# adamnelsonarcher/BB-OCR

Measured on AMD Instinct MI355X. Metric: book-page images/sec end-to-end (detect+recognize) @1280x960, higher is better.
Workload: dtype fp16

## Files before the change

bb-ocr_amd/csrc/conv_mfma.hip:

```cpp
#include "common.h"
#include "kernels.h"
#include <type_traits>
#include <utility>

__device__ __forceinline__ void lds_dma16(const void* gptr, const void* lds) {
    const unsigned la = (unsigned)(size_t)(const __attribute__((address_space(3))) void*)lds;
    asm volatile("s_mov_b32 m0, %1\n\ts_nop 0\n\tglobal_load_lds_dwordx4 %0, off" ::"v"(gptr), "s"(la) : "memory");
}

template <int EL, int MF, bool ADDUP = false>
__device__ __forceinline__ void conv_epilogue(const ConvArgs& a, f32x4 (&acc)[MF][4], int n, int nt, int oy0, int ox0, int wm, int wn, int fpr,
                                              int lane, int BN, int sub = 1, int sph = 0, int spw = 0) {
    const int g = lane >> 4, pl = lane & 15;
    const int cout0 = nt * BN + wn * 64 + g * 8;
    if (a.tail) {
        const float* tw = a.tail;
        const typename El<EL>::v8 w1f = *(const typename El<EL>::v8*)(a.tail_frag + lane * 8);
        float cb[8], b1r[4], w2a[4], w2b[4];
#pragma unroll
        for (int i = 0; i < 8; ++i) cb[i] = a.bias[(g & 1) * 8 + i];
#pragma unroll
        for (int r = 0; r < 4; ++r) { b1r[r] = tw[4 * g + r]; w2a[r] = tw[16 + 4 * g + r]; w2b[r] = tw[32 + 4 * g + r]; }
        const float b20 = tw[48], b21 = tw[49];
#pragma unroll
// ... 221 lines not shown
                            *(u32x4*)(op) = lo;
                            if (run1) *(u32x4*)(op + 32) = hi;
                        }
                    };
                    if (a.split_off) {
                        float mh[16], ml[16];
                        split_hi_lo(m, mh, ml);
                        store_pooled(mh, 0);
                        store_pooled(ml, a.split_off);
                    } else {
                        store_pooled(m, 0);
                    }
                } else {
                    store_frag(a.pool_out, prow, a.pool_cs, xb, POW, py < POH, m, false);
                }
            }
        }
    };
    if (fpr == 1) pooled(std::integral_constant<int, 1>{});
    else if (fpr == 2) pooled(std::integral_constant<int, 2>{});
    else pooled(std::integral_constant<int, 4>{});
}

template <int EL, int MF>
__device__ __forceinline__ void conv_epilogue_pool2x2_lean(const ConvArgs& a, f32x4 (&acc)[MF][4], int n, int oy0, int ox0, int wm, int lane,
                                                           int cout_base = 0) {
    static_assert(MF % 2 == 0, "fragment f and f + 1 are the two rows of a pooling window");
    const int g = lane >> 4, pl = lane & 15, odd = pl & 1;
    const int cout0 = cout_base + g * 8;
    const float sc = a.acc_scale;
    const float floor_v = (a.relu_out || a.pool_relu) ? 0.f : -__builtin_inff();
    float bsel[8];
#pragma unroll
    for (int q = 0; q < 2; ++q) {
        const f32x4 b4 = *(const f32x4*)(a.bias + cout0 + odd * 32 + q * 4);
        bsel[q * 4 + 0] = b4[0]; bsel[q * 4 + 1] = b4[1]; bsel[q * 4 + 2] = b4[2]; bsel[q * 4 + 3] = b4[3];
    }
    const int POH = a.OH >> 1, POW = a.OW >> 1;
    const int px = (ox0 + pl) >> 1;
#pragma unroll
    for (int f = 0; f < MF; f += 2) {
        const int py = (oy0 + wm * MF + f) >> 1;
        float o[8];
#pragma unroll
        for (int i = 0; i < 8; ++i) {
            const int i1 = 8 + i;
            float q0 = fmaxf(acc[f][i >> 2][i & 3], acc[f + 1][i >> 2][i & 3]);
            float q1 = fmaxf(acc[f][i1 >> 2][i1 & 3], acc[f + 1][i1 >> 2][i1 & 3]);
            q0 = fmaxf(q0, __int_as_float(__builtin_amdgcn_update_dpp(0, __float_as_int(q0), 0xB1 , 0xF, 0xF, true)));
            q1 = fmaxf(q1, __int_as_float(__builtin_amdgcn_update_dpp(0, __float_as_int(q1), 0xB1, 0xF, 0xF, true)));
            o[i] = fmaxf(fmaf(odd ? q1 : q0, sc, bsel[i]), floor_v);
        }
        const u32x4 pk = {El<EL>::pack2(o[0], o[1]), El<EL>::pack2(o[2], o[3]), El<EL>::pack2(o[4], o[5]), El<EL>::pack2(o[6], o[7])};
        uint16_t* op = (uint16_t*)a.pool_out + ((size_t)(n * POH + py) * POW + px) * a.pool_cs + cout0 + odd * 32;
        if (py < POH && px < POW) *(u32x4*)op = pk;
    }
}

template <int EL, int MF>
__device__ __forceinline__ void conv_epilogue_plain_lean(const ConvArgs& a, f32x4 (&acc)[MF][4], int n, int nt, int oy0, int ox0, int wm, int wn,
                                                         int fpr, int lane, int BN) {
    typedef short s16x2_t __attribute__((ext_vector_type(2)));
    const int g = lane >> 4, pl = lane & 15;
    const int cout0 = nt * BN + wn * 64 + g * 8;
    float bs[16];
#pragma unroll
    for (int h = 0; h < 2; ++h)
#pragma unroll
        for (int q = 0; q < 2; ++q) {
            const f32x4 b4 = *(const f32x4*)(a.bias + cout0 + h * 32 + q * 4);
            bs[h * 8 + q * 4 + 0] = b4[0]; bs[h * 8 + q * 4 + 1] = b4[1]; bs[h * 8 + q * 4 + 2] = b4[2]; bs[h * 8 + q * 4 + 3] = b4[3];
        }
    const bool relu = a.relu_out != 0;
    const bool inside = oy0 + a.TH <= a.OH && ox0 + a.TW <= a.OW;
    const s16x2_t z2 = {0, 0};
    const size_t lane_off = (size_t)(pl & 7) * a.out_cs + cout0 + (pl >> 3) * 32;
#pragma unroll
    for (int f = 0; f < MF; ++f) {
        const int F = wm * MF + f;
// ... 239 lines not shown
                typename El<EL>::v8 bq[MF];
#pragma unroll
                for (int f = 0; f < MF; ++f) bq[f] = *(const typename El<EL>::v8*)(pb + frag_off[f]);
#pragma unroll
                for (int f = 0; f < MF; ++f) {
#pragma unroll
                    for (int j = 0; j < 4; ++j) acc[f][j] = El<EL>::mfma(af[j], bq[f], acc[f][j]);
                }
                __builtin_amdgcn_sched_group_barrier(0x100, 4 + MF, 0);
                __builtin_amdgcn_sched_group_barrier(0x008, 4 * MF, 0);
                if (more) {
                    if (a.ntaps >= 3) stage_patch_store(c + 1, tap);
                    else if (tap == a.ntaps - 1) store_part(c + 1, P0{});
                }
                __syncthreads();
                if (++kx == a.KW) { kx = 0; ++ky; }
            }
        }
    }

    conv_epilogue<EL, MF>(a, acc, n, nt, oy0, ox0, wm, wn, fpr, lane, BN);
}

template <int EL, int WM, int WN, int MF, int NPB, int RING, int NPS = NPB * 64, bool FUSE1 = false, int NF = 4, int EPI = 0, int KS = 3>
__global__ void __launch_bounds__(WM * WN * 64, 2) conv3x3_dma_kernel(const ConvArgs a) {
    constexpr int NTAP = KS * KS, PAD = KS == 3 ? 1 : 0;
    static_assert((KS == 3 || KS == 2) && (KS == 3 || (!FUSE1 && EPI == 0)), "kernel size");
    constexpr int NW = WM * WN, NT = NW * 64, BN = WN * 64;
    static_assert(NW == 4, "one wave per 8-channel group of the patch");
    constexpr int WBUF = BN * 64, WPIECES = WBUF / 16, WPT = WPIECES / NT;
    static_assert(WPIECES % NT == 0 && (RING == 3 || RING == 4), "uniform DMA issue");
    constexpr int NP = NPS, PSLOTS = NTAP + 1 - RING;
    constexpr int PPER = (NPB + PSLOTS - 1) / PSLOTS;
    static_assert(NPS <= NPB * 64 && NPS > (NPB - 1) * 64 && NPS % 4 == 0, "patch size");
    static_assert(PSLOTS >= 1 && PPER * PSLOTS >= NPB, "patch does not fit the DMA schedule");
    extern __shared__ __attribute__((aligned(16))) unsigned char smem[];
    unsigned char* const wbuf = smem;
    unsigned char* const pbuf = smem + RING * WBUF;
    constexpr int patch_bytes = NP * 64;

    const int tid = threadIdx.x;
    const int lane = tid & 63;
    const int wave = __builtin_amdgcn_readfirstlane(tid >> 6);
    const int wm = wave / WN, wn = wave % WN;
    const int sub = a.sub;
    const int nk = a.nchunks * NTAP;
    const int fpr = FUSE1 ? 1 : a.TW >> 4;
    const int PW = FUSE1 ? 18 : a.PW;

    const int tile = xcd_remap(blockIdx.x, gridDim.x);
    struct Geo {
        int n, nt, oy0, ox0, sph, spw;
        const unsigned char* wsrc;
    };
    auto geom = [&](int id, Geo& g) {
        g.nt = id % a.ntiles_n;
        id /= a.ntiles_n;
        const int tx = id % a.tiles_x;
        id /= a.tiles_x;
        const int ty = id % a.tiles_y;
        int n = id / a.tiles_y;
        g.sph = 0; g.spw = 0;
        g.n = n;
        g.oy0 = ty * a.TH; g.ox0 = tx * a.TW;
        g.wsrc = (const unsigned char*)a.wpk + (size_t)g.nt * nk * WBUF;
    };
    int spix[NPB];
    const int pw_magic = (65536 + a.PW - 1) / a.PW;
    const int stack_magic = ((1 << 20) + a.stack) / (a.stack + 1);
    auto geom_pix = [&](const Geo& g) {
        const int iy0 = g.oy0 - PAD, ix0 = g.ox0 - PAD;
#pragma unroll
        for (int pb = 0; pb < NPB; ++pb) {
            const int pix = pb * 64 + lane;
            const int py = (pix * pw_magic) >> 16, px = pix - py * a.PW;
            int ly = iy0 + py;
            const int lx = ix0 + px;
            int sph = 0, spw = 0;
            bool rowok = ly >= 0;
            if (sub > 1) {
                const int vy = ly < 0 ? 0 : ly;
                const int q = (vy * stack_magic) >> 20;
                ly = vy - q * (a.stack + 1);
                sph = q / sub;
                spw = q - sph * sub;
                rowok = rowok && ly < a.stack && q < sub * sub;
            }
            const int iy = ly * sub + sph, ix = lx * sub + spw;
            spix[pb] = (py < a.PH && rowok && iy < a.H && lx >= 0 && ix < a.W) ? (g.n * a.H + iy) * a.W + ix : -1;
        }
    };
    Geo cur;
    geom(tile, cur);
    if constexpr (!FUSE1) geom_pix(cur);

    auto issue_p = [&](int sp, int chunk, int par, auto pb_c) {
        constexpr int pb = decltype(pb_c)::value;
        const int c = chunk * 32;
        const bool s0 = c < a.C0;
        const uint16_t* src = s0 ? a.in0 : a.in1;
        const int cs = s0 ? a.in0_cs : a.in1_cs;
        const int cb = (s0 ? c : c - a.C0) + wave * 8;
        const uint16_t* gp = sp >= 0 ? src + (size_t)sp * cs + cb : (const uint16_t*)a.zero;
        if ((pb + 1) * 64 <= NPS || pb * 64 + lane < NPS)
            lds_dma16(gp, pbuf + par * patch_bytes + (wave * NP + pb * 64) * 16);
    };
    auto issue_w = [&](const unsigned char* slice, int slot) {
#pragma unroll
        for (int p0 = 0; p0 < WPIECES; p0 += NT) lds_dma16(slice + (size_t)(p0 + tid) * 16, wbuf + slot * WBUF + (p0 + wave * 64) * 16);
    };
    int frag_off[MF];
#pragma unroll
    for (int f = 0; f < MF; ++f) {
        const int F = wm * MF + f;
        const int fr = F / fpr, fc = F - fr * fpr;
        frag_off[f] = (fr * PW + fc * 16) * 16;
    }
    const int lane_patch_off = ((lane >> 4) * NP + (lane & 15)) * 16;
    const int lane_w_off = wn * 4 * 1024 + lane * 16;

    struct Sched {
        static constexpr int pcnt(int tap) {
            if (FUSE1 || tap >= PSLOTS) return 0;
            const int base = NPB / PSLOTS, extra = NPB % PSLOTS;
            return base + (tap < extra ? 1 : 0);
        }
        static constexpr int pfirst(int tap) { int s = 0; for (int t = 0; t < tap; ++t) s += pcnt(t); return s; }
        static constexpr int wcnt(bool more, int tap) { return (more || tap < NTAP - (RING - 1)) ? WPT : 0; }
        static constexpr int younger(bool more, int tap) {
            int nv = wcnt(more, tap) + (more ? pcnt(tap) : 0);
            for (int back = 1; back <= RING - 2; ++back) {
                const int t = tap - back;
                const bool m = t >= 0 ? more : true;
                const int tt = t >= 0 ? t : t + NTAP;
                const int pc = m ? pcnt(tt) : 0;
                nv += (back == RING - 2) ? pc : (wcnt(m, tt) + pc);
            }
            return nv;
        }
    };
    static_assert(FUSE1 || Sched::pfirst(NTAP) == NPB, "patch DMA schedule must cover the patch");

#pragma unroll
    for (int i = 0; i < RING - 1; ++i)
        if (i < nk) issue_w(cur.wsrc + (size_t)i * WBUF, i);
    if constexpr (!FUSE1) {
        [&]<int... PB>(std::integer_sequence<int, PB...>) { (issue_p(spix[PB], 0, 0, std::integral_constant<int, PB>{}), ...); }(std::make_integer_sequence<int, NPB>{});
    } else {
        static_assert(!FUSE1 || (RING == 3 && BN == 64 && NPS == 324), "fused conv1_1 producer: 16x16 tiles, 3-deep ring of 4 KB slices");
        u32x2* const rgbp = (u32x2*)(wbuf + 2 * WBUF);
        const uint8_t* rgb = (const uint8_t*)a.in0;
        const float m0 = 0.485f * 255.0f, m1 = 0.456f * 255.0f, m2 = 0.406f * 255.0f;
        const float s0 = 0.229f * 255.0f, s1 = 0.224f * 255.0f, s2 = 0.225f * 255.0f;
        static_assert(NT == 256, "two patch pixels per thread");
        int pq[2];
        bool on_canvas[2];
        unsigned int cr[2], cg[2], cb[2];
#pragma unroll
        for (int it = 0; it < 2; ++it) {
            const int p = tid + it * NT;
            const int py = p / 20, px = p - py * 20;
            const int iy = cur.oy0 - 2 + py, ix = cur.ox0 - 2 + px;
            pq[it] = p;
            on_canvas[it] = p < 400 && iy >= 0 && iy < a.H && ix >= 0 && ix < a.W;
            const bool on_page = on_canvas[it] && iy < a.rgb_H && ix < a.rgb_W;
            const uint8_t* q = rgb + (on_page ? ((size_t)(cur.n * a.rgb_H + iy) * a.rgb_W + ix) * 3 : (size_t)cur.n * a.rgb_H * a.rgb_W * 3);
            cr[it] = q[0]; cg[it] = q[1]; cb[it] = q[2];
            if (!on_page) { cr[it] = 0u; cg[it] = 0u; cb[it] = 0u; }
        }
        typename El<EL>::v8 w1[4];
#pragma unroll
        for (int j = 0; j < 4; ++j) w1[j] = *(const typename El<EL>::v8*)(a.c11_w + ((size_t)j * 64 + lane) * 8);
        const int g = lane >> 4, pl = lane & 15;
        f32x4 b1[4];
#pragma unroll
        for (int h = 0; h < 2; ++h)
#pragma unroll
            for (int q4 = 0; q4 < 2; ++q4) b1[h * 2 + q4] = *(const f32x4*)(a.c11_b + h * 32 + g * 8 + q4 * 4);
        __builtin_amdgcn_sched_barrier(0);
#pragma unroll
        for (int it = 0; it < 2; ++it) {
            if (pq[it] < 400) {
                u32x2 v = {0u, 0u};
                if (on_canvas[it]) {
                    v[0] = El<EL>::pack2(((float)cr[it] - m0) / s0, ((float)cg[it] - m1) / s1);
                    v[1] = El<EL>::pack2(((float)cb[it] - m2) / s2, 0.f);
                }
                rgbp[pq[it]] = v;
            }
        }
        __syncthreads();
        auto frag_geo = [&](int fi, int& pp, int& py, int& px) {
            pp = fi * 16 + pl;
            py = pp / 18;
            px = pp - py * 18;
        };
#pragma unroll
        for (int b3 = 0; b3 < 2; ++b3) {
            typename El<EL>::v8 bfr[3];
            int pps[3], pys[3], pxs[3];
#pragma unroll
            for (int q = 0; q < 3; ++q) {
                const int fi = wave + (b3 * 3 + q) * NW;
                frag_geo(fi < 21 ? fi : 20, pps[q], pys[q], pxs[q]);
                const int pc = pps[q] < 324 ? pys[q] * 20 + pxs[q] : 0;
                const int t0 = 2 * g, t1 = t0 + 1;
                const u32x2 a0 = rgbp[pc + (t0 / 3) * 20 + (t0 % 3)];
                const u32x2 a1 = rgbp[pc + (t1 / 3) * 20 + (t1 % 3)];
                const u32x2 t8 = rgbp[pc + 2 * 20 + 2];
                const unsigned int x = g == 0 ? (t8[0] << 16) : (g == 1 ? (t8[1] << 16) : 0u);
                const unsigned int y = g == 0 ? (t8[0] & 0xffff0000u) : 0u;
                bfr[q] = __builtin_bit_cast(typename El<EL>::v8, (u32x4){a0[0], a0[1] | x, a1[0], a1[1] | y});
            }
            f32x4 d[3][4];
#pragma unroll
            for (int q = 0; q < 3; ++q)
#pragma unroll
                for (int j = 0; j < 4; ++j) d[q][j] = El<EL>::mfma(w1[j], bfr[q], b1[j]);
#pragma unroll
            for (int q = 0; q < 3; ++q) {
                const int fi = wave + (b3 * 3 + q) * NW;
                const int pp = pps[q];
                const int iy = cur.oy0 - 1 + pys[q], ix = cur.ox0 - 1 + pxs[q];
                const bool inside = iy >= 0 && iy < a.H && ix >= 0 && ix < a.W;
                const float cap = inside ? __builtin_inff() : 0.f;
                if (fi < 21 && pp < 324) {
#pragma unroll
                    for (int h = 0; h < 2; ++h) {
                        u32x4 o;
#pragma unroll
                        for (int i = 0; i < 4; ++i) {
                            const int k = h * 8 + i * 2;
                            const float x0 = __builtin_amdgcn_fmed3f(d[q][k >> 2][k & 3], 0.f, cap), x1 = __builtin_amdgcn_fmed3f(d[q][(k + 1) >> 2][(k + 1) & 3], 0.f, cap);
                            o[i] = El<EL>::pack2(x0, x1);
                        }
                        *(u32x4*)(pbuf + h * patch_bytes + (g * NP + pp) * 16) = o;
                    }
                }
            }
        }
    }
    asm volatile("s_waitcnt vmcnt(0) lgkmcnt(0)\n\ts_barrier" ::: "memory");

    int wslot = 0, par = 0;
    const unsigned char* wp = cur.wsrc + (size_t)(RING - 1) * WBUF;
    f32x4 acc[MF][4];
#pragma unroll
    for (int f = 0; f < MF; ++f)
#pragma unroll
        for (int j = 0; j < 4; ++j) acc[f][j] = (f32x4){0.f, 0.f, 0.f, 0.f};
    static_assert(MF % 2 == 0 && MF >= 4, "B fragments are scheduled in pairs, four ahead");
    typename El<EL>::v8 pre[4];
    auto step = [&](auto tap_c, auto more_c, int c) {
        constexpr int tap = decltype(tap_c)::value;
        constexpr bool MORE = decltype(more_c)::value;
        constexpr int ky = tap / KS, kx = tap % KS;
        const unsigned char* wb = wbuf + wslot * WBUF + lane_w_off;
        const unsigned char* pb = pbuf + par * patch_bytes + lane_patch_off + (ky * PW + kx) * 16;
        typename El<EL>::v8 af[NF], bq[MF];
#pragma unroll
        for (int j = 0; j < NF; ++j) af[j] = *(const typename El<EL>::v8*)(wb + j * 1024);
        if constexpr (tap == 0) {
#pragma unroll
            for (int f = 0; f < 4; ++f) bq[f] = *(const typename El<EL>::v8*)(pb + frag_off[f]);
// ... 31 lines not shown
            __builtin_amdgcn_sched_barrier(0);
        }
        asm volatile("s_waitcnt vmcnt(%0)\n\ts_barrier" ::"n"(Sched::younger(MORE, tap)) : "memory");
        wslot = wslot + 1 == RING ? 0 : wslot + 1;
    };
    auto relu_patch = [&](int c) {
        if (!((c * 32 < a.C0) ? a.relu_in0 : a.relu_in1)) return;
        const s16x8 z = {0, 0, 0, 0, 0, 0, 0, 0};
        s16x8* pp = (s16x8*)(pbuf + par * patch_bytes);
#pragma unroll
        for (int i = 0; i < (NP * 4 + NT - 1) / NT; ++i) {
            const int k = tid + i * NT;
            if ((i + 1) * NT <= NP * 4 || k < NP * 4) pp[k] = __builtin_elementwise_max(pp[k], z);
        }
        asm volatile("s_waitcnt lgkmcnt(0)\n\ts_barrier" ::: "memory");
    };
    auto chunk = [&](auto more_c, int c) {
        relu_patch(c);
        [&]<int... T>(std::integer_sequence<int, T...>) { (step(std::integral_constant<int, T>{}, more_c, c), ...); }(std::make_integer_sequence<int, NTAP>{});
        par ^= 1;
    };
    for (int c = 0; c + 1 < a.nchunks; ++c) chunk(std::true_type{}, c);
    chunk(std::false_type{}, a.nchunks - 1);
    if constexpr (FUSE1) conv_epilogue_pool2x2_lean<EL, MF>(a, acc, cur.n, cur.oy0, cur.ox0, wm, lane);
    else if constexpr (EPI == 1) conv_epilogue_post1x1<EL, MF>(a, acc, cur.n, cur.oy0, cur.ox0, wm, fpr, lane);
    else if constexpr (KS == 3 && NF == 4) {
        if (a.lean == 1) conv_epilogue_plain_lean<EL, MF>(a, acc, cur.n, cur.nt, cur.oy0, cur.ox0, wm, wn, fpr, lane, BN);
        else if (a.lean == 3) conv_epilogue_pool2x2_lean<EL, MF>(a, acc, cur.n, cur.oy0, cur.ox0, wm, lane, cur.nt * BN + wn * 64);
        else conv_epilogue<EL, MF>(a, acc, cur.n, cur.nt, cur.oy0, cur.ox0, wm, wn, fpr, lane, BN, sub, cur.sph, cur.spw);
    } else conv_epilogue<EL, MF>(a, acc, cur.n, cur.nt, cur.oy0, cur.ox0, wm, wn, fpr, lane, BN, sub, cur.sph, cur.spw);
}

template <int EL, int NCH, bool DB, int NF = 2, bool LEAN = false>
__global__ void __launch_bounds__(256, 2) conv3x3_resw_kernel(const ConvArgs a) {
    static_assert(NF == 2 || (NF == 4 && NCH == 1), "resident weights");
    constexpr int MF = 4, NP = 324, NPB = 6, NK = NCH * 9;
    constexpr int WSL = NF * 1024;
    constexpr int PCH = NP * 64;
    constexpr int NBUF = DB ? 2 : 1;
    extern __shared__ __attribute__((aligned(16))) unsigned char smem[];
    unsigned char* const wres = smem;
    unsigned char* const pbuf = smem + NK * WSL;
    const int tid = threadIdx.x, lane = tid & 63;
    const int wave = __builtin_amdgcn_readfirstlane(tid >> 6);
    const int wm = wave;
    const int ntiles = a.N * a.tiles_x * a.tiles_y;
    {
        const unsigned char* wsrc = (const unsigned char*)a.wpk;
// ... 97 lines not shown
            if (next < ntiles) issue_patch(next, 0);
        }
        if constexpr (LEAN) conv_epilogue_pool2x2_lean<EL, MF>(a, acc, n, ty * 16, tx * 16, wm, lane);
        else conv_epilogue<EL, MF>(a, acc, n, 0, ty * 16, tx * 16, wm, 0, 1, lane, 64);
        if constexpr (DB) buf ^= 1;
    }
}

template <int EL>
static hipError_t launch_resw(const ConvArgs& a, hipStream_t s) {
    const int ntiles = a.N * a.tiles_x * a.tiles_y;
    const int ncu = device_cus();
    auto go = [&](auto kern, size_t smem, int per_cu, LdsOptIn& attr) -> hipError_t {
        if (hipError_t e = lds_opt_in(attr, (const void*)kern, smem); e != hipSuccess) return e;
        const int grid = ntiles < ncu * per_cu ? ntiles : ncu * per_cu;
        hipLaunchKernelGGL(kern, dim3(grid), dim3(256), smem, s, a);
        return hipGetLastError();
    };
    constexpr size_t P = 324 * 64, W1 = 9 * 2048, W2 = 18 * 2048;
    static LdsOptIn at[3];
    if (a.cout_store == 64) return go(conv3x3_resw_kernel<EL, 1, true, 4, true>, 9 * 4096 + 2 * P, 2, at[2]);
    if (a.nchunks == 1) return go(conv3x3_resw_kernel<EL, 1, true>, W1 + 2 * P, 2, at[0]);
    return go(conv3x3_resw_kernel<EL, 2, false>, W2 + 2 * P, 2, at[1]);
}

template <int EL>
__global__ void __launch_bounds__(256, 2) conv3x3_up4_kernel(const ConvArgs a) {
    constexpr int MF = 4, NF = 2, NP = 324, NK = 18, WSL = NF * 1024, PCH = NP * 64, NFRAG = 21;
    typedef typename El<EL>::v8 v8;
    extern __shared__ __attribute__((aligned(16))) unsigned char smem[];
    unsigned char* const wres = smem;
    unsigned char* const pbuf = smem + NK * WSL;
    const int tid = threadIdx.x, lane = tid & 63;
    const int wave = __builtin_amdgcn_readfirstlane(tid >> 6);
    const int g = lane >> 4, pl = lane & 15;
    const int ntiles = a.N * a.tiles_x * a.tiles_y;
    {
        const unsigned char* wsrc = (const unsigned char*)a.wpk;
#pragma unroll
        for (int k2 = 0; k2 < NK / 2; ++k2) {
            const int ks = k2 * 2 + (wave >> 1);
            lds_dma16(wsrc + (size_t)ks * 4096 + (size_t)(tid & 127) * 16, wres + ks * WSL + (wave & 1) * 1024);
        }
    }
    v8 w1[4][4];
#pragma unroll
// ... 284 lines not shown
                            if (cout < p.Cout && cin < p.Cin) v = w[((size_t)cout * p.Cin + cin) * ntaps + tap];
                            out[o++] = f32_to_el_host(p.el, v);
                        }
                    }
                }
}

template <int EL, int WM, int WN, int MF, int PITER>
static hipError_t launch_one(const ConvArgs& a, size_t smem, int grid, hipStream_t s) {
    auto k = conv_mfma_kernel<EL, WM, WN, MF, PITER>;
    static LdsOptIn attr;
    if (hipError_t e = lds_opt_in(attr, (const void*)k, smem); e != hipSuccess) return e;
    hipLaunchKernelGGL(k, dim3(grid), dim3(WM * WN * 64), smem, s, a);
    return hipGetLastError();
}

template <int EL, int WM, int WN, int MF, int PITER>
static hipError_t launch_cfg(const ConvArgs& a, int grid, hipStream_t s) {
    const size_t smem = (size_t)2 * WN * 64 * 64 + (size_t)2 * a.NP * 64;
    if (smem > 160 * 1024) return hipErrorInvalidValue;
    return launch_one<EL, WM, WN, MF, PITER>(a, smem, grid, s);
}

template <int EL, int WM, int WN, int MF, int NPB, int RING, int NPS = NPB * 64, bool FUSE1 = false, int NF = 4, int EPI = 0, int KS = 3>
static hipError_t launch_dma_one(ConvArgs a, int grid, hipStream_t s) {
    auto k = conv3x3_dma_kernel<EL, WM, WN, MF, NPB, RING, NPS, FUSE1, NF, EPI, KS>;
    const size_t smem_max = (size_t)RING * WN * 64 * 64 + (size_t)2 * NPS * 64;
    const size_t smem = (a.nchunks == 1 && !FUSE1) ? smem_max - (size_t)NPS * 64 : smem_max;
    static LdsOptIn attr;
    if (hipError_t e = lds_opt_in(attr, (const void*)k, smem_max); e != hipSuccess) return e;
    {
        a.lean = 0;
        const bool plain = !FUSE1 && EPI == 0 && KS == 3 && NF == 4 && a.sub == 1 && !a.out_f32 && !a.tail && !a.split_off && !a.addup && !a.post_w &&
                           a.acc_scale == 1.f && a.cout_store == a.ntiles_n * WN * 64 && a.out_cs % 8 == 0;
        if (plain && a.pool_mode == 0 && a.out) a.lean = 1;
        else if (plain && a.pool_mode == 1 && !a.store_full && a.TH == 16 && a.TW == 16 && a.pool_out) a.lean = 3;
    }
    hipLaunchKernelGGL(k, dim3(grid), dim3(WM * WN * 64), smem, s, a);
    return hipGetLastError();
}

template <int EL, int WM, int WN, int MF>
static hipError_t launch_dma(const ConvArgs& a, int npb, int grid, hipStream_t s) {
    if constexpr (WN == 1) {
        if (a.c11_w) {
            if (!(npb == 6 && a.PH == 18 && a.PW == 18 && a.TH == 16 && a.TW == 16 && a.nchunks == 2 && a.sub == 1)) return hipErrorInvalidValue;
            if (!(a.pool_mode == 1 && !a.store_full && !a.split_off && !a.out_f32 && !a.tail && a.cout_store == 64 && a.ntiles_n == 1 && a.acc_scale > 0.f))
                return hipErrorInvalidValue;
            return launch_dma_one<EL, WM, WN, MF, 6, 3, 324, true>(a, grid, s);
        }
    }
    if (a.post_w) {
        if constexpr (WN == 1)
            if (npb == 6 && a.PH == 18 && a.PW == 18 && a.cout_store == 64 && a.ntiles_n == 1 && a.sub == 1 && !a.pool_mode && !a.split_off &&
                !a.out_f32 && !a.tail && !a.addup)
                return launch_dma_one<EL, WM, WN, MF, 6, 3, 324, false, 4, 1>(a, grid, s);
        return hipErrorNotSupported;
    }
    if constexpr (WN == 1) {
        if (npb == 6 && a.PH * a.PW == 324) {
            if (a.cout_store <= 32 && a.nchunks <= 2 && a.sub == 1 && !a.C1 && !a.pool_mode && a.TH == 16 && a.TW == 16 && a.ntiles_n == 1)
                return launch_resw<EL>(a, s);
            if (a.cout_store == 64 && a.nchunks == 1 && a.sub == 1 && !a.C1 && a.pool_mode == 1 && !a.store_full && !a.split_off && !a.out_f32 &&
                !a.tail && !a.relu_in0 && a.TH == 16 && a.TW == 16 && a.ntiles_n == 1 && a.acc_scale > 0.f)
                return launch_resw<EL>(a, s);
            if (a.cout_store <= 32) return launch_dma_one<EL, WM, WN, MF, 6, 3, 324, false, 2>(a, grid, s);
            return launch_dma_one<EL, WM, WN, MF, 6, 3, 324>(a, grid, s);
        }
        if (npb == 6) return launch_dma_one<EL, WM, WN, MF, 6, 3>(a, grid, s);
    } else if (npb == 6) {
        const size_t wb = (size_t)WN * 64 * 64, pb = (size_t)2 * npb * 64 * 64;
        return 4 * wb + pb <= 80 * 1024 ? launch_dma_one<EL, WM, WN, MF, 6, 4>(a, grid, s) : launch_dma_one<EL, WM, WN, MF, 6, 3>(a, grid, s);
    }
    if (npb == 7) return launch_dma_one<EL, WM, WN, MF, 7, 3>(a, grid, s);
    return hipErrorInvalidValue;
}

int conv_plan_bn(int Cout) {
    return Cout > 64 ? 128 : 64;
}

template <int EL>
static hipError_t launch_conv_el(const ConvPlan& p, ConvArgs a, hipStream_t s) {
    const int BN = p.BN;
    constexpr int NWV = 4;
    constexpr int BM = 256;
    a.KH = p.KH; a.KW = p.KW; a.pad_h = p.pad_h; a.pad_w = p.pad_w; a.dil = p.dil;
    a.OH = a.H + 2 * p.pad_h - (p.KH - 1) * p.dil;
    a.OW = a.W + 2 * p.pad_w - (p.KW - 1) * p.dil;
// ... 49 lines not shown
            const long long tiles = (long long)cdiv(a.OH, th) * cdiv(a.OW, tw);
            const long long cost = tiles * ((long long)BM * a.ntaps + 2LL * np);
            if (best < 0 || cost < best) { best = cost; a.TH = th; a.TW = tw; a.PH = ph; a.PW = pw; a.NP = np; }
        }
        if (best < 0) return hipErrorInvalidValue;
    }
    a.tiles_x = cdiv(a.OW, a.TW);
    a.tiles_y = cdiv(a.OH, a.TH);
    a.ntiles_n = p.Cout_pad / BN;
    a.nchunks = p.Cin_pad / 32;
    if (a.C0 + a.C1 != p.Cin_pad || (a.C0 & 31) || (a.C1 & 31)) return hipErrorInvalidValue;
    if ((a.in0_cs & 7) || (a.C1 && (a.in1_cs & 7)) || (a.out_cs & (a.out_f32 ? 3 : 7)) || (a.cout_store & 15)) return hipErrorInvalidValue;
    a.wpk = p.d_w;
    a.bias = p.d_b;
    const long long grid_ll = (long long)a.N * a.tiles_x * a.tiles_y * a.ntiles_n;
    if (grid_ll <= 0 || grid_ll > 0x7fffffffLL) return hipErrorInvalidValue;
    const int grid = (int)grid_ll;
    if (a.addup && !(p.KH == 1 && p.KW == 1 && a.zero && !a.pool_mode && !a.out_f32 && !a.tail && a.cout_store % 64 == 0 &&
                     a.cout_store == p.Cout_pad))
        return hipErrorInvalidValue;
    if (p.KH == 1 && p.KW == 1 && p.pad_h == 0 && p.pad_w == 0 && a.zero && !a.pool_mode)
        return BN == 256 ? launch_dma1x1<EL, 2, 4, 8>(a, s) : (BN == 128 ? launch_dma1x1<EL, 2, 2, 8>(a, s) : launch_dma1x1<EL, 4, 1, 4>(a, s));
    if (dma2x2)
        return BN == 128 ? launch_dma_one<EL, 2, 2, 8, 6, 4, 384, false, 4, 0, 2>(a, grid, s) : launch_dma_one<EL, 4, 1, 4, 6, 3, 384, false, 4, 0, 2>(a, grid, s);
    if (p.KH == 3 && p.KW == 3 && p.dil == 1 && p.pad_h == 1 && p.pad_w == 1 && a.zero) {
        const int npb = cdiv(a.PH * a.PW, 64);
        if (npb == 6 || npb == 7) {
            a.NP = npb * 64;
            return BN == 128 ? launch_dma<EL, 2, 2, 8>(a, npb, grid, s) : launch_dma<EL, 4, 1, 4>(a, npb, grid, s);
        }
    }
    if (a.c11_w || a.addup || a.post_w) return hipErrorNotSupported;
    const int piter = cdiv(a.NP / 16, NWV);
    if (BN == 128) return piter <= 4 ? launch_cfg<EL, 2, 2, 8, 4>(a, grid, s) : (piter <= 8 ? launch_cfg<EL, 2, 2, 8, 8>(a, grid, s) : launch_cfg<EL, 2, 2, 8, 16>(a, grid, s));
    if (BN == 64) return piter <= 4 ? launch_cfg<EL, 4, 1, 4, 4>(a, grid, s) : (piter <= 8 ? launch_cfg<EL, 4, 1, 4, 8>(a, grid, s) : launch_cfg<EL, 4, 1, 4, 16>(a, grid, s));
    return hipErrorInvalidValue;
}

hipError_t launch_conv(const ConvPlan& p, ConvArgs a, hipStream_t s) {
    a.acc_scale = p.acc_scale;
    if (a.split_off && (a.out_f32 || a.tail || a.addup || p.el != 1)) return hipErrorInvalidValue;
    return p.el ? launch_conv_el<1>(p, a, s) : launch_conv_el<0>(p, a, s);
}
```

Measured before the change: 959.8.

## Add persistent weight-resident fused conv1_1+conv1_2 kernel with producer/consumer wave groups

Replaces the FUSE1 path of the DMA conv kernel, which ran fused conv1_1+conv1_2+pool, with a persistent kernel launched one block per CU. Each block loads all conv1_2 weights into LDS once. Two 4-wave groups then alternate phases, one producing the conv1_1 patch from RGB while the other runs the conv1_2 MFMA loop and pool epilogue, with the next tile's RGB loads prefetched under the math. This targets the repeated per-tile weight streaming and the serialized produce-then-multiply structure, at the cost of a large LDS footprint, occupancy of one block per CU, and possible load imbalance across the persistent tile streams.

Measured after the change: 960.6 (median of 3 runs). No clear change (+0.1%).

```diff
diff --git a/bb-ocr_amd/csrc/conv_mfma.hip b/bb-ocr_amd/csrc/conv_mfma.hip
--- a/bb-ocr_amd/csrc/conv_mfma.hip
+++ b/bb-ocr_amd/csrc/conv_mfma.hip
@@ -267,20 +267,22 @@
     else pooled(std::integral_constant<int, 4>{});
 }
 
+__device__ __forceinline__ void pool2x2_lean_bias(const ConvArgs& a, int lane, int cout_base, float (&bsel)[8]) {
+    const int g = lane >> 4, odd = lane & 1;
+#pragma unroll
+    for (int q = 0; q < 2; ++q) {
+        const f32x4 b4 = *(const f32x4*)(a.bias + cout_base + g * 8 + odd * 32 + q * 4);
+        bsel[q * 4 + 0] = b4[0]; bsel[q * 4 + 1] = b4[1]; bsel[q * 4 + 2] = b4[2]; bsel[q * 4 + 3] = b4[3];
+    }
+}
 template <int EL, int MF>
 __device__ __forceinline__ void conv_epilogue_pool2x2_lean(const ConvArgs& a, f32x4 (&acc)[MF][4], int n, int oy0, int ox0, int wm, int lane,
-                                                           int cout_base = 0) {
+                                                           int cout_base, const float (&bsel)[8]) {
     static_assert(MF % 2 == 0, "fragment f and f + 1 are the two rows of a pooling window");
     const int g = lane >> 4, pl = lane & 15, odd = pl & 1;
     const int cout0 = cout_base + g * 8;
     const float sc = a.acc_scale;
     const float floor_v = (a.relu_out || a.pool_relu) ? 0.f : -__builtin_inff();
-    float bsel[8];
-#pragma unroll
-    for (int q = 0; q < 2; ++q) {
-        const f32x4 b4 = *(const f32x4*)(a.bias + cout0 + odd * 32 + q * 4);
-        bsel[q * 4 + 0] = b4[0]; bsel[q * 4 + 1] = b4[1]; bsel[q * 4 + 2] = b4[2]; bsel[q * 4 + 3] = b4[3];
-    }
     const int POH = a.OH >> 1, POW = a.OW >> 1;
     const int px = (ox0 + pl) >> 1;
 #pragma unroll
@@ -300,6 +302,13 @@
         uint16_t* op = (uint16_t*)a.pool_out + ((size_t)(n * POH + py) * POW + px) * a.pool_cs + cout0 + odd * 32;
         if (py < POH && px < POW) *(u32x4*)op = pk;
     }
+}
+template <int EL, int MF>
+__device__ __forceinline__ void conv_epilogue_pool2x2_lean(const ConvArgs& a, f32x4 (&acc)[MF][4], int n, int oy0, int ox0, int wm, int lane,
+                                                           int cout_base = 0) {
+    float bsel[8];
+    pool2x2_lean_bias(a, lane, cout_base, bsel);
+    conv_epilogue_pool2x2_lean<EL, MF>(a, acc, n, oy0, ox0, wm, lane, cout_base, bsel);
 }
 
 template <int EL, int MF>
@@ -585,10 +594,10 @@
     conv_epilogue<EL, MF>(a, acc, n, nt, oy0, ox0, wm, wn, fpr, lane, BN);
 }
 
-template <int EL, int WM, int WN, int MF, int NPB, int RING, int NPS = NPB * 64, bool FUSE1 = false, int NF = 4, int EPI = 0, int KS = 3>
+template <int EL, int WM, int WN, int MF, int NPB, int RING, int NPS = NPB * 64, int NF = 4, int EPI = 0, int KS = 3>
 __global__ void __launch_bounds__(WM * WN * 64, 2) conv3x3_dma_kernel(const ConvArgs a) {
     constexpr int NTAP = KS * KS, PAD = KS == 3 ? 1 : 0;
-    static_assert((KS == 3 || KS == 2) && (KS == 3 || (!FUSE1 && EPI == 0)), "kernel size");
+    static_assert((KS == 3 || KS == 2) && (KS == 3 || EPI == 0), "kernel size");
     constexpr int NW = WM * WN, NT = NW * 64, BN = WN * 64;
     static_assert(NW == 4, "one wave per 8-channel group of the patch");
     constexpr int WBUF = BN * 64, WPIECES = WBUF / 16, WPT = WPIECES / NT;
@@ -608,8 +617,8 @@
     const int wm = wave / WN, wn = wave % WN;
     const int sub = a.sub;
     const int nk = a.nchunks * NTAP;
-    const int fpr = FUSE1 ? 1 : a.TW >> 4;
-    const int PW = FUSE1 ? 18 : a.PW;
+    const int fpr = a.TW >> 4;
+    const int PW = a.PW;
 
     const int tile = xcd_remap(blockIdx.x, gridDim.x);
     struct Geo {
@@ -655,7 +664,7 @@
     };
     Geo cur;
     geom(tile, cur);
-    if constexpr (!FUSE1) geom_pix(cur);
+    geom_pix(cur);
 
     auto issue_p = [&](int sp, int chunk, int par, auto pb_c) {
         constexpr int pb = decltype(pb_c)::value;
@@ -684,7 +693,7 @@
 
     struct Sched {
         static constexpr int pcnt(int tap) {
-            if (FUSE1 || tap >= PSLOTS) return 0;
+            if (tap >= PSLOTS) return 0;
             const int base = NPB / PSLOTS, extra = NPB % PSLOTS;
             return base + (tap < extra ? 1 : 0);
         }
@@ -702,107 +711,12 @@
             return nv;
         }
     };
-    static_assert(FUSE1 || Sched::pfirst(NTAP) == NPB, "patch DMA schedule must cover the patch");
+    static_assert(Sched::pfirst(NTAP) == NPB, "patch DMA schedule must cover the patch");
 
 #pragma unroll
     for (int i = 0; i < RING - 1; ++i)
         if (i < nk) issue_w(cur.wsrc + (size_t)i * WBUF, i);
-    if constexpr (!FUSE1) {
-        [&]<int... PB>(std::integer_sequence<int, PB...>) { (issue_p(spix[PB], 0, 0, std::integral_constant<int, PB>{}), ...); }(std::make_integer_sequence<int, NPB>{});
-    } else {
-        static_assert(!FUSE1 || (RING == 3 && BN == 64 && NPS == 324), "fused conv1_1 producer: 16x16 tiles, 3-deep ring of 4 KB slices");
-        u32x2* const rgbp = (u32x2*)(wbuf + 2 * WBUF);
-        const uint8_t* rgb = (const uint8_t*)a.in0;
-        const float m0 = 0.485f * 255.0f, m1 = 0.456f * 255.0f, m2 = 0.406f * 255.0f;
-        const float s0 = 0.229f * 255.0f, s1 = 0.224f * 255.0f, s2 = 0.225f * 255.0f;
-        static_assert(NT == 256, "two patch pixels per thread");
-        int pq[2];
-        bool on_canvas[2];
-        unsigned int cr[2], cg[2], cb[2];
-#pragma unroll
-        for (int it = 0; it < 2; ++it) {
-            const int p = tid + it * NT;
-            const int py = p / 20, px = p - py * 20;
-            const int iy = cur.oy0 - 2 + py, ix = cur.ox0 - 2 + px;
-            pq[it] = p;
-            on_canvas[it] = p < 400 && iy >= 0 && iy < a.H && ix >= 0 && ix < a.W;
-            const bool on_page = on_canvas[it] && iy < a.rgb_H && ix < a.rgb_W;
-            const uint8_t* q = rgb + (on_page ? ((size_t)(cur.n * a.rgb_H + iy) * a.rgb_W + ix) * 3 : (size_t)cur.n * a.rgb_H * a.rgb_W * 3);
-            cr[it] = q[0]; cg[it] = q[1]; cb[it] = q[2];
-            if (!on_page) { cr[it] = 0u; cg[it] = 0u; cb[it] = 0u; }
-        }
-        typename El<EL>::v8 w1[4];
-#pragma unroll
-        for (int j = 0; j < 4; ++j) w1[j] = *(const typename El<EL>::v8*)(a.c11_w + ((size_t)j * 64 + lane) * 8);
-        const int g = lane >> 4, pl = lane & 15;
-        f32x4 b1[4];
-#pragma unroll
-        for (int h = 0; h < 2; ++h)
-#pragma unroll
-            for (int q4 = 0; q4 < 2; ++q4) b1[h * 2 + q4] = *(const f32x4*)(a.c11_b + h * 32 + g * 8 + q4 * 4);
-        __builtin_amdgcn_sched_barrier(0);
-#pragma unroll
-        for (int it = 0; it < 2; ++it) {
-            if (pq[it] < 400) {
-                u32x2 v = {0u, 0u};
-                if (on_canvas[it]) {
-                    v[0] = El<EL>::pack2(((float)cr[it] - m0) / s0, ((float)cg[it] - m1) / s1);
-                    v[1] = El<EL>::pack2(((float)cb[it] - m2) / s2, 0.f);
-                }
-                rgbp[pq[it]] = v;
-            }
-        }
-        __syncthreads();
-        auto frag_geo = [&](int fi, int& pp, int& py, int& px) {
-            pp = fi * 16 + pl;
-            py = pp / 18;
-            px = pp - py * 18;
-        };
-#pragma unroll
-        for (int b3 = 0; b3 < 2; ++b3) {
-            typename El<EL>::v8 bfr[3];
-            int pps[3], pys[3], pxs[3];
-#pragma unroll
-            for (int q = 0; q < 3; ++q) {
-                const int fi = wave + (b3 * 3 + q) * NW;
-                frag_geo(fi < 21 ? fi : 20, pps[q], pys[q], pxs[q]);
-                const int pc = pps[q] < 324 ? pys[q] * 20 + pxs[q] : 0;
-                const int t0 = 2 * g, t1 = t0 + 1;
-                const u32x2 a0 = rgbp[pc + (t0 / 3) * 20 + (t0 % 3)];
-                const u32x2 a1 = rgbp[pc + (t1 / 3) * 20 + (t1 % 3)];
-                const u32x2 t8 = rgbp[pc + 2 * 20 + 2];
-                const unsigned int x = g == 0 ? (t8[0] << 16) : (g == 1 ? (t8[1] << 16) : 0u);
-                const unsigned int y = g == 0 ? (t8[0] & 0xffff0000u) : 0u;
-                bfr[q] = __builtin_bit_cast(typename El<EL>::v8, (u32x4){a0[0], a0[1] | x, a1[0], a1[1] | y});
-            }
-            f32x4 d[3][4];
-#pragma unroll
-            for (int q = 0; q < 3; ++q)
-#pragma unroll
-                for (int j = 0; j < 4; ++j) d[q][j] = El<EL>::mfma(w1[j], bfr[q], b1[j]);
-#pragma unroll
-            for (int q = 0; q < 3; ++q) {
-                const int fi = wave + (b3 * 3 + q) * NW;
-                const int pp = pps[q];
-                const int iy = cur.oy0 - 1 + pys[q], ix = cur.ox0 - 1 + pxs[q];
-                const bool inside = iy >= 0 && iy < a.H && ix >= 0 && ix < a.W;
-                const float cap = inside ? __builtin_inff() : 0.f;
-                if (fi < 21 && pp < 324) {
-#pragma unroll
-                    for (int h = 0; h < 2; ++h) {
-                        u32x4 o;
-#pragma unroll
-                        for (int i = 0; i < 4; ++i) {
-                            const int k = h * 8 + i * 2;
-                            const float x0 = __builtin_amdgcn_fmed3f(d[q][k >> 2][k & 3], 0.f, cap), x1 = __builtin_amdgcn_fmed3f(d[q][(k + 1) >> 2][(k + 1) & 3], 0.f, cap);
-                            o[i] = El<EL>::pack2(x0, x1);
-                        }
-                        *(u32x4*)(pbuf + h * patch_bytes + (g * NP + pp) * 16) = o;
-                    }
-                }
-            }
-        }
-    }
+    [&]<int... PB>(std::integer_sequence<int, PB...>) { (issue_p(spix[PB], 0, 0, std::integral_constant<int, PB>{}), ...); }(std::make_integer_sequence<int, NPB>{});
     asm volatile("s_waitcnt vmcnt(0) lgkmcnt(0)\n\ts_barrier" ::: "memory");
 
     int wslot = 0, par = 0;
@@ -880,8 +794,7 @@
     };
     for (int c = 0; c + 1 < a.nchunks; ++c) chunk(std::true_type{}, c);
     chunk(std::false_type{}, a.nchunks - 1);
-    if constexpr (FUSE1) conv_epilogue_pool2x2_lean<EL, MF>(a, acc, cur.n, cur.oy0, cur.ox0, wm, lane);
-    else if constexpr (EPI == 1) conv_epilogue_post1x1<EL, MF>(a, acc, cur.n, cur.oy0, cur.ox0, wm, fpr, lane);
+    if constexpr (EPI == 1) conv_epilogue_post1x1<EL, MF>(a, acc, cur.n, cur.oy0, cur.ox0, wm, fpr, lane);
     else if constexpr (KS == 3 && NF == 4) {
         if (a.lean == 1) conv_epilogue_plain_lean<EL, MF>(a, acc, cur.n, cur.nt, cur.oy0, cur.ox0, wm, wn, fpr, lane, BN);
         else if (a.lean == 3) conv_epilogue_pool2x2_lean<EL, MF>(a, acc, cur.n, cur.oy0, cur.ox0, wm, lane, cur.nt * BN + wn * 64);
@@ -1025,6 +938,221 @@
     if (a.cout_store == 64) return go(conv3x3_resw_kernel<EL, 1, true, 4, true>, 9 * 4096 + 2 * P, 2, at[2]);
     if (a.nchunks == 1) return go(conv3x3_resw_kernel<EL, 1, true>, W1 + 2 * P, 2, at[0]);
     return go(conv3x3_resw_kernel<EL, 2, false>, W2 + 2 * P, 2, at[1]);
+}
+
+template <int EL>
+__global__ void __launch_bounds__(512, 1) conv1_2_resident_kernel(const ConvArgs a) {
+    constexpr int MF = 4, NP = 324, PCH = NP * 64, NK = 18, WBYTES = NK * 4096, PBUF = 2 * PCH, RGBB = 400 * 8;
+    static_assert(WBYTES + 2 * PBUF + 2 * RGBB <= 160 * 1024, "LDS");
+    extern __shared__ __attribute__((aligned(16))) unsigned char smem[];
+    const int tid = threadIdx.x, lane = tid & 63;
+    const int wave = __builtin_amdgcn_readfirstlane(tid >> 6);
+    const int grp = wave >> 2, wm = wave & 3, gtid = tid & 255;
+    unsigned char* const wres = smem;
+    unsigned char* const pbuf = smem + WBYTES + grp * PBUF;
+    u32x2* const rgbp = (u32x2*)(smem + WBYTES + 2 * PBUF + grp * RGBB);
+#pragma unroll
+    for (int i = 0; i < WBYTES / 8192; ++i)
+        lds_dma16((const unsigned char*)a.wpk + (size_t)i * 8192 + (size_t)tid * 16, wres + i * 8192 + wave * 1024);
+
+    const int ntiles = a.N * a.tiles_x * a.tiles_y;
+    const int nstreams = 2 * gridDim.x;
+    const int stream0 = 2 * xcd_remap(blockIdx.x, gridDim.x);
+    auto stream_len = [&](int s) { return s < ntiles ? (ntiles - 1 - s) / nstreams + 1 : 0; };
+    const int n0 = stream_len(stream0), n1 = stream_len(stream0 + 1);
+    const int nmine = grp ? n1 : n0;
+    const int nph = n1 == n0 ? 2 * n0 + 1 : 2 * n0;
+    struct Geo { int n, oy0, ox0; };
+    auto geom = [&](int it) {
+        int id = stream0 + grp + it * nstreams;
+        const int tx = id % a.tiles_x;
+        id /= a.tiles_x;
+        return Geo{id / a.tiles_y, (id % a.tiles_y) * 16, tx * 16};
+    };
+
+    const uint8_t* rgb = (const uint8_t*)a.in0;
+    int one = 1;
+    asm volatile("" : "+s"(one));
+    struct Stage {
+        bool on_canvas[2], on_page[2];
+        unsigned int cr[2], cg[2], cb[2];
+    };
+    auto stage_load = [&](const Geo& t, Stage& st) {
+#pragma unroll
+        for (int it = 0; it < 2; ++it) {
+            const int p = gtid + it * 256;
+            const int py = p / 20, px = p - py * 20;
+            const int iy = t.oy0 - 2 + py, ix = t.ox0 - 2 + px;
+            st.on_canvas[it] = (p < 400) & (iy >= 0) & (iy < a.H) & (ix >= 0) & (ix < a.W);
+            const bool on_page = st.on_canvas[it] & (iy < a.rgb_H) & (ix < a.rgb_W);
+            st.on_page[it] = on_page;
+            const uint8_t* q = rgb + ((size_t)(t.n * a.rgb_H + (on_page ? iy : 0)) * a.rgb_W + (on_page ? ix : 0)) * 3;
+            st.cr[it] = q[0]; st.cg[it] = q[one]; st.cb[it] = q[2 * one];
+        }
+    };
+    auto stage_store = [&](const Stage& st) {
+        const float m0 = 0.485f * 255.0f, m1 = 0.456f * 255.0f, m2 = 0.406f * 255.0f;
+        const float s0 = 0.229f * 255.0f, s1 = 0.224f * 255.0f, s2 = 0.225f * 255.0f;
+#pragma unroll
+        for (int it = 0; it < 2; ++it) {
+            const int p = gtid + it * 256;
+            if (p < 400) {
+                u32x2 v = {0u, 0u};
+                if (st.on_canvas[it]) {
+                    const unsigned int r = st.on_page[it] ? (unsigned int)st.cr[it] : 0u, gg = st.on_page[it] ? (unsigned int)st.cg[it] : 0u, b = st.on_page[it] ? (unsigned int)st.cb[it] : 0u;
+                    v[0] = El<EL>::pack2(((float)r - m0) / s0, ((float)gg - m1) / s1);
+                    v[1] = El<EL>::pack2(((float)b - m2) / s2, 0.f);
+                }
+                rgbp[p] = v;
+            }
+        }
+    };
+
+    const int g = lane >> 4, pl = lane & 15;
+    typename El<EL>::v8 w1[4];
+#pragma unroll
+    for (int j = 0; j < 4; ++j) w1[j] = *(const typename El<EL>::v8*)(a.c11_w + ((size_t)j * 64 + lane) * 8);
+    f32x4 b1[4];
+#pragma unroll
+    for (int h = 0; h < 2; ++h)
+#pragma unroll
+        for (int q4 = 0; q4 < 2; ++q4) b1[h * 2 + q4] = *(const f32x4*)(a.c11_b + h * 32 + g * 8 + q4 * 4);
+    float bsel[8];
+    pool2x2_lean_bias(a, lane, 0, bsel);
+
+    auto produce = [&](const Geo& t) {
+#pragma unroll
+        for (int b3 = 0; b3 < 2; ++b3) {
+            typename El<EL>::v8 bfr[3];
+            int pps[3], pys[3], pxs[3];
+#pragma unroll
+            for (int q = 0; q < 3; ++q) {
+                const int fi = wm + (b3 * 3 + q) * 4;
+                pps[q] = (fi < 21 ? fi : 20) * 16 + pl;
+                pys[q] = pps[q] / 18;
+                pxs[q] = pps[q] - pys[q] * 18;
+                const int pc = pps[q] < 324 ? pys[q] * 20 + pxs[q] : 0;
+                const int t0 = 2 * g, t1 = t0 + 1;
+                const u32x2 a0 = rgbp[pc + (t0 / 3) * 20 + (t0 % 3)];
+                const u32x2 a1 = rgbp[pc + (t1 / 3) * 20 + (t1 % 3)];
+                const u32x2 t8 = rgbp[pc + 2 * 20 + 2];
+                const unsigned int x = g == 0 ? (t8[0] << 16) : (g == 1 ? (t8[1] << 16) : 0u);
+                const unsigned int y = g == 0 ? (t8[0] & 0xffff0000u) : 0u;
+                bfr[q] = __builtin_bit_cast(typename El<EL>::v8, (u32x4){a0[0], a0[1] | x, a1[0], a1[1] | y});
+            }
+            f32x4 d[3][4];
+#pragma unroll
+            for (int q = 0; q < 3; ++q)
+#pragma unroll
+                for (int j = 0; j < 4; ++j) d[q][j] = El<EL>::mfma(w1[j], bfr[q], b1[j]);
+#pragma unroll
+            for (int q = 0; q < 3; ++q) {
+                const int fi = wm + (b3 * 3 + q) * 4;
+                const int pp = pps[q];
+                const int iy = t.oy0 - 1 + pys[q], ix = t.ox0 - 1 + pxs[q];
+                const bool inside = iy >= 0 && iy < a.H && ix >= 0 && ix < a.W;
+                const float cap = inside ? __builtin_inff() : 0.f;
+                if (fi < 21 && pp < 324) {
+#pragma unroll
+                    for (int h = 0; h < 2; ++h) {
+                        u32x4 o;
+#pragma unroll
+                        for (int i = 0; i < 4; ++i) {
+                            const int k = h * 8 + i * 2;
+                            const float x0 = __builtin_amdgcn_fmed3f(d[q][k >> 2][k & 3], 0.f, cap), x1 = __builtin_amdgcn_fmed3f(d[q][(k + 1) >> 2][(k + 1) & 3], 0.f, cap);
+                            o[i] = El<EL>::pack2(x0, x1);
+                        }
+                        *(u32x4*)(pbuf + h * PCH + (g * NP + pp) * 16) = o;
+                    }
+                }
+            }
+        }
+    };
+
+    const unsigned char* const wl = wres + lane * 16;
+    const unsigned char* const pl0 = pbuf + (g * NP + pl + wm * MF * 18) * 16;
+    auto multiply = [&](int it) {
+        const Geo t = geom(it);
+        const bool has_next = it + 1 < nmine;
+        Stage st;
+        if (has_next) stage_load(geom(it + 1), st);
+        __builtin_amdgcn_sched_barrier(0);
+        f32x4 acc[MF][4];
+#pragma unroll
+        for (int f = 0; f < MF; ++f)
+#pragma unroll
+            for (int j = 0; j < 4; ++j) acc[f][j] = (f32x4){0.f, 0.f, 0.f, 0.f};
+        typename El<EL>::v8 af[4], bq[MF];
+        auto rdA = [&](auto ks_c, typename El<EL>::v8(&x)[4]) {
+            constexpr int ks = decltype(ks_c)::value;
+#pragma unroll
+            for (int j = 0; j < 4; ++j) x[j] = *(const typename El<EL>::v8*)(wl + ks * 4096 + j * 1024);
+        };
+        auto rdB = [&](auto ks_c, auto f_c, typename El<EL>::v8(&x)[MF]) {
+            constexpr int ks = decltype(ks_c)::value, f = decltype(f_c)::value, c = ks / 9, tap = ks % 9;
+            x[f] = *(const typename El<EL>::v8*)(pl0 + c * PCH + ((tap / 3) * 18 + tap % 3 + f * 18) * 16);
+        };
+        using I0 = std::integral_constant<int, 0>; using I1 = std::integral_constant<int, 1>;
+        using I2 = std::integral_constant<int, 2>; using I3 = std::integral_constant<int, 3>;
+        rdA(I0{}, af);
+        rdB(I0{}, I0{}, bq); rdB(I0{}, I1{}, bq); rdB(I0{}, I2{}, bq); rdB(I0{}, I3{}, bq);
+        auto step = [&](auto ks_c) {
+            constexpr int ks = decltype(ks_c)::value;
+            using NX = std::integral_constant<int, (ks + 1 < NK ? ks + 1 : ks)>;
+            typename El<EL>::v8 afn[4], bqn[MF];
+            __builtin_amdgcn_sched_barrier(0);
+#pragma unroll
+            for (int f = 0; f < 2; ++f)
+#pragma unroll
+                for (int j = 0; j < 4; ++j) acc[f][j] = El<EL>::mfma(af[j], bq[f], acc[f][j]);
+            __builtin_amdgcn_sched_barrier(0);
+            if constexpr (ks + 1 < NK) { rdA(NX{}, afn); rdB(NX{}, I0{}, bqn); rdB(NX{}, I1{}, bqn); }
+            __builtin_amdgcn_sched_barrier(0);
+#pragma unroll
+            for (int f = 2; f < 4; ++f)
+#pragma unroll
+                for (int j = 0; j < 4; ++j) acc[f][j] = El<EL>::mfma(af[j], bq[f], acc[f][j]);
+            __builtin_amdgcn_sched_barrier(0);
+            if constexpr (ks + 1 < NK) {
+                rdB(NX{}, I2{}, bqn); rdB(NX{}, I3{}, bqn);
+#pragma unroll
+                for (int j = 0; j < 4; ++j) { af[j] = afn[j]; bq[j] = bqn[j]; }
+            }
+        };
+        [&]<int... KS>(std::integer_sequence<int, KS...>) { (step(std::integral_constant<int, KS>{}), ...); }(std::make_integer_sequence<int, NK>{});
+        __builtin_amdgcn_sched_barrier(0);
+        if (has_next) {
+            asm volatile("" : "+v"(st.cr[0]), "+v"(st.cr[1]), "+v"(st.cg[0]), "+v"(st.cg[1]), "+v"(st.cb[0]), "+v"(st.cb[1]));
+            stage_store(st);
+        }
+        conv_epilogue_pool2x2_lean<EL, MF>(a, acc, t.n, t.oy0, t.ox0, wm, lane, 0, bsel);
+    };
+
+    if (nmine > 0) {
+        Stage st;
+        stage_load(geom(0), st);
+        stage_store(st);
+    }
+    __builtin_amdgcn_s_waitcnt(0x0070);
+    asm volatile("s_waitcnt vmcnt(0) lgkmcnt(0)\n\ts_barrier" ::: "memory");
+    for (int ph = 0; ph < nph; ++ph) {
+        const int itp = ph >> 1, itm = (ph - 1) >> 1;
+        if ((ph & 1) == grp) {
+            if (itp < nmine) produce(geom(itp));
+        } else if (ph >= 1 && itm < nmine) {
+            multiply(itm);
+        }
+        if (ph + 1 < nph) asm volatile("s_waitcnt lgkmcnt(0)\n\ts_barrier" ::: "memory");
+    }
+}
+
+template <int EL>
+static hipError_t launch_c12_resident(const ConvArgs& a, hipStream_t s) {
+    constexpr size_t smem = 18 * 4096 + 2 * (2 * 324 * 64) + 2 * (400 * 8);
+    static LdsOptIn attr;
+    if (hipError_t e = lds_opt_in(attr, (const void*)conv1_2_resident_kernel<EL>, smem); e != hipSuccess) return e;
+    hipLaunchKernelGGL(conv1_2_resident_kernel<EL>, dim3(device_cus()), dim3(512), smem, s, a);
+    return hipGetLastError();
 }
 
 template <int EL>
@@ -1355,16 +1483,16 @@
     return launch_one<EL, WM, WN, MF, PITER>(a, smem, grid, s);
 }
 
-template <int EL, int WM, int WN, int MF, int NPB, int RING, int NPS = NPB * 64, bool FUSE1 = false, int NF = 4, int EPI = 0, int KS = 3>
+template <int EL, int WM, int WN, int MF, int NPB, int RING, int NPS = NPB * 64, int NF = 4, int EPI = 0, int KS = 3>
 static hipError_t launch_dma_one(ConvArgs a, int grid, hipStream_t s) {
-    auto k = conv3x3_dma_kernel<EL, WM, WN, MF, NPB, RING, NPS, FUSE1, NF, EPI, KS>;
+    auto k = conv3x3_dma_kernel<EL, WM, WN, MF, NPB, RING, NPS, NF, EPI, KS>;
     const size_t smem_max = (size_t)RING * WN * 64 * 64 + (size_t)2 * NPS * 64;
-    const size_t smem = (a.nchunks == 1 && !FUSE1) ? smem_max - (size_t)NPS * 64 : smem_max;
+    const size_t smem = a.nchunks == 1 ? smem_max - (size_t)NPS * 64 : smem_max;
     static LdsOptIn attr;
     if (hipError_t e = lds_opt_in(attr, (const void*)k, smem_max); e != hipSuccess) return e;
     {
         a.lean = 0;
-        const bool plain = !FUSE1 && EPI == 0 && KS == 3 && NF == 4 && a.sub == 1 && !a.out_f32 && !a.tail && !a.split_off && !a.addup && !a.post_w &&
+        const bool plain = EPI == 0 && KS == 3 && NF == 4 && a.sub == 1 && !a.out_f32 && !a.tail && !a.split_off && !a.addup && !a.post_w &&
                            a.acc_scale == 1.f && a.cout_store == a.ntiles_n * WN * 64 && a.out_cs % 8 == 0;
         if (plain && a.pool_mode == 0 && a.out) a.lean = 1;
         else if (plain && a.pool_mode == 1 && !a.store_full && a.TH == 16 && a.TW == 16 && a.pool_out) a.lean = 3;
@@ -1380,14 +1508,14 @@
             if (!(npb == 6 && a.PH == 18 && a.PW == 18 && a.TH == 16 && a.TW == 16 && a.nchunks == 2 && a.sub == 1)) return hipErrorInvalidValue;
             if (!(a.pool_mode == 1 && !a.store_full && !a.split_off && !a.out_f32 && !a.tail && a.cout_store == 64 && a.ntiles_n == 1 && a.acc_scale > 0.f))
                 return hipErrorInvalidValue;
-            return launch_dma_one<EL, WM, WN, MF, 6, 3, 324, true>(a, grid, s);
+            return launch_c12_resident<EL>(a, s);
         }
     }
     if (a.post_w) {
         if constexpr (WN == 1)
             if (npb == 6 && a.PH == 18 && a.PW == 18 && a.cout_store == 64 && a.ntiles_n == 1 && a.sub == 1 && !a.pool_mode && !a.split_off &&
                 !a.out_f32 && !a.tail && !a.addup)
-                return launch_dma_one<EL, WM, WN, MF, 6, 3, 324, false, 4, 1>(a, grid, s);
+                return launch_dma_one<EL, WM, WN, MF, 6, 3, 324, 4, 1>(a, grid, s);
         return hipErrorNotSupported;
     }
     if constexpr (WN == 1) {
@@ -1397,7 +1525,7 @@
             if (a.cout_store == 64 && a.nchunks == 1 && a.sub == 1 && !a.C1 && a.pool_mode == 1 && !a.store_full && !a.split_off && !a.out_f32 &&
                 !a.tail && !a.relu_in0 && a.TH == 16 && a.TW == 16 && a.ntiles_n == 1 && a.acc_scale > 0.f)
                 return launch_resw<EL>(a, s);
-            if (a.cout_store <= 32) return launch_dma_one<EL, WM, WN, MF, 6, 3, 324, false, 2>(a, grid, s);
+            if (a.cout_store <= 32) return launch_dma_one<EL, WM, WN, MF, 6, 3, 324, 2>(a, grid, s);
             return launch_dma_one<EL, WM, WN, MF, 6, 3, 324>(a, grid, s);
         }
         if (npb == 6) return launch_dma_one<EL, WM, WN, MF, 6, 3>(a, grid, s);
@@ -1493,7 +1621,7 @@
     if (p.KH == 1 && p.KW == 1 && p.pad_h == 0 && p.pad_w == 0 && a.zero && !a.pool_mode)
         return BN == 256 ? launch_dma1x1<EL, 2, 4, 8>(a, s) : (BN == 128 ? launch_dma1x1<EL, 2, 2, 8>(a, s) : launch_dma1x1<EL, 4, 1, 4>(a, s));
     if (dma2x2)
-        return BN == 128 ? launch_dma_one<EL, 2, 2, 8, 6, 4, 384, false, 4, 0, 2>(a, grid, s) : launch_dma_one<EL, 4, 1, 4, 6, 3, 384, false, 4, 0, 2>(a, grid, s);
+        return BN == 128 ? launch_dma_one<EL, 2, 2, 8, 6, 4, 384, 4, 0, 2>(a, grid, s) : launch_dma_one<EL, 4, 1, 4, 6, 3, 384, 4, 0, 2>(a, grid, s);
     if (p.KH == 3 && p.KW == 3 && p.dil == 1 && p.pad_h == 1 && p.pad_w == 1 && a.zero) {
         const int npb = cdiv(a.PH * a.PW, 64);
         if (npb == 6 || npb == 7) {
```
